# ziniuwan/maed

Hardware: AMD Instinct MI355X
Metric: video-clips/sec (BxT frames) train step (higher is better)
Workload: dtype bf16

## Files before the change

include/maed_hip.h:

```cpp
#ifndef MAED_HIP_H
#define MAED_HIP_H

#include <stddef.h>
#include <stdint.h>

#ifdef __cplusplus
extern "C" {
#endif

typedef enum { MAED_F32 = 0, MAED_BF16 = 1,
               MAED_F32X3 = 2, MAED_F32X6 = 3,
               MAED_F32X1 = 4 } maed_dtype;

typedef enum {
    MAED_OK = 0,
    MAED_ERR_ARG = -1,
    MAED_ERR_SHAPE = -2,
    MAED_ERR_ALIGN = -3,
    MAED_ERR_LAUNCH = -4,
    MAED_ERR_UNSUPPORTED = -5
} maed_status;

typedef enum {
    MAED_EPI_STORE = 0,
// ... 21 lines not shown
const char* maed_last_error(void);
int maed_version(void);

typedef enum {
    MAED_OPT_F32_MATMUL = 0,
    MAED_OPT_SIDE_STREAM = 1,
    MAED_OPT_TN_TARGET_WGS = 2,
    MAED_OPT_ABLATE = 3,
    MAED_OPT_GN_BWD_ONEPASS = 4,
    MAED_OPT_F32_BWD_X1 = 5,
    MAED_OPT_ST_FUSED = 6,
    MAED_OPT_CONV3X3_ROWS_WGS = 7,
    MAED_OPT_STEM_WGRAD_WGS = 8,
    MAED_OPT_LBS_FRAMES = 9,
    MAED_OPT_TN_DMA = 10,
    MAED_OPT_X3_PLANES = 11,
    MAED_OPT_X3_PLANES_LN = 12,
    MAED_OPT_SK = 13,
    MAED_OPT_SK_GRID = 14,
    MAED_OPT_TN_SK = 15,
    MAED_OPT_CONV3X3_NARROW_WGS = 16,
    MAED_OPT_CONV3X3_FRAME = 17,
    MAED_OPT_CONV3X3_WGRAD_TAPS = 18,
    MAED_OPT_COUNT
} maed_option;
int maed_init(int device);
int maed_device_faults(void);
int maed_device_faults_clear(void);
int maed_set_option(int key, int value);
int maed_get_option(int key);

int maed_layernorm_fwd(const float* x, int64_t x_row_stride, const float* gamma, const float* beta,
                       void* y, int dtype, float* mean, float* rstd,
                       int64_t rows, int C, float eps, void* stream);
int maed_layernorm_bwd(const void* dy, int dtype, const float* x, int64_t x_row_stride,
                       const float* gamma, const float* mean, const float* rstd,
                       const float* dres_in, float* dx_out, void* dx_twin, float* dgamma, float* dbeta,
                       int64_t rows, int C, void* stream);

int maed_gemm_nt(const void* A, int64_t lda, const void* B, int64_t ldb,
                 int64_t M, int64_t N, int64_t K, int dtype, int epilogue,
                 const float* bias, void* out, int64_t ldo, void* out2,
                 const void* aux, int64_t ldaux, int splitk, int impl, void* stream);

int maed_gemm_nt_planes(const void* a_hi, const void* a_lo, int64_t lda, const void* b_hi, const void* b_lo, int64_t ldb, int64_t M, int64_t N, int64_t K,
                        int epilogue, const float* bias, void* out, int64_t ldo, void* out2_bf16, const void* aux, int64_t ldaux, void* out_hi, void* out_lo,
// ... 162 lines not shown

int maed_loss_accl_fwd_bwd(const float* pred_kp3d, const float* gt_kp3d, int N, int T, float weight, double* loss, float* d_kp3d, void* stream);

typedef struct {
    const float* w;
    float* gw;
    const void* gout;
    int64_t dst_off;
    int64_t dst_t_off;
    int32_t O, I, KHW, fstart;
    int32_t gout_f32;
    int32_t pad_;
} maed_ws_conv;
int maed_weight_std_fwd(const void* conv_table, int n_convs, int n_filters, void* out, int dtype, float* stats, float eps, int transpose_tiles, void* stream);
int maed_weight_std_bwd(const void* conv_table, int n_convs, int n_filters, int dtype, const float* stats, float eps, void* stream);
int maed_groupnorm_fwd(const void* x, const void* residual, const float* gamma, const float* beta, void* y, double* sums,
                       uint8_t* relu_mask, int N, int HW, int C, float eps, int relu, int dtype, int sums_zeroed, void* stream);
int maed_groupnorm_fwd_twin(const void* x, const void* residual, const float* gamma, const float* beta, void* y, double* sums,
                            uint8_t* relu_mask, int N, int HW, int C, float eps, int relu, int sums_zeroed, void* twin_x, void* twin_y, void* stream);
#define MAED_GN_SYNC_WORDS 80
int maed_groupnorm_bwd(const void* x, const uint8_t* relu_mask, const void* dy, const double* sums, const float* gamma, const float* beta,
                       void* dx, void* dres, float* dgamma, float* dbeta, float* ab_scratch, int N, int HW, int C, float eps,
                       int relu, int dtype, int ab_zeroed, uint32_t* frame_sync, void* aux_stream, void* stream);
typedef struct { const float* ab; float* dgamma; float* dbeta; int N; int C; } maed_gn_affine_item;
int maed_gn_affine_grad_batch(const maed_gn_affine_item* items, int count, void* stream);

int maed_maxpool3s2_same_fwd(const void* x, void* y, uint8_t* idx, int N, int H, int W, int C, int dtype, void* stream);
int maed_maxpool3s2_same_bwd(const void* dy, const uint8_t* idx, void* dx, int N, int H, int W, int C, int dtype, void* stream);
int maed_gn_relu_maxpool3s2_fwd(const void* x, const float* gamma, const float* beta, void* y, uint8_t* idx, double* sums, int N, int H, int W, int C, float eps,
                                int dtype, int sums_zeroed, void* stream);
int maed_groupnorm_dual_fwd(const void* x, const float* gamma, const float* beta, double* sums, const void* res, const float* gamma2, const float* beta2,
                            double* sums2, void* y, uint8_t* relu_mask, int N, int HW, int C, float eps, float eps2, int dtype, int sums_zeroed,
                            int sums2_zeroed, void* stream);

int maed_stem_input(const float* x, void* y, int N, int C, int H, int W, int pad_top, int pad_bottom, int pad_left, int pad_right, int c_stride, int dtype,
                    void* stream);

int maed_conv3x3_wgrad_rows64_scratch_floats(int F, int H, int W, int Cin, int Cout);
int maed_conv3x3_wgrad_rows64(const void* dy, const void* x, float* dW, void* scratch, int F, int H, int W, int dtype, void* stream);

int maed_conv3x3_wgrad_taps_scratch_floats(int F, int H, int W, int Cin, int Cout, int stride, int Ho, int Wo);
int maed_conv3x3_wgrad_taps(const void* dy, const void* x, const void* zero_page, float* dW, void* scratch, int F, int H, int W, int Cin, int Cout, int stride,
                            int pad_top, int pad_left, int Ho, int Wo, int dtype, void* stream);

int maed_stem7x7s2_supported(int H, int W);
int maed_stem7x7s2_fwd(const void* xp, const void* w, void* wimg, void* y, double* gn_sums, int F, int H, int W, int dtype, void* stream);
// ... 81 lines not shown
```

maed_amd/_lib.py:

```python
import ctypes as C
import os

HERE = os.path.dirname(os.path.abspath(__file__))
LIB_PATH = os.environ.get("MAED_HIP_LIB") or os.path.join(HERE, "libmaed_hip.so")

F32, BF16 = 0, 1
F32X3, F32X6, F32X1 = 2, 3, 4
EPI_STORE, EPI_GELU, EPI_RESID_F32, EPI_MUL_DGELU, EPI_ATOMIC_F32, EPI_STORE_F32, EPI_TANH, EPI_ADD = range(8)
EPI_RESID_DROP_F32, EPI_GELU_DROP, EPI_MUL_DGELU_DROP = 8, 9, 10
DROP_GOLD, DROP_SITE = 0x9E3779B97F4A7C15, 0xD1B54A32D192ED03
IMPL_AUTO, IMPL_VALU, IMPL_MFMA = 0, 1, 2
IMPL_MFMA_256 = 6
IMPL_MFMA_LONG = 5
IMPL_MFMA_SK = 10
IMPL_X3, IMPL_X6, IMPL_X1 = 7, 8, 9
(OPT_F32_MATMUL, OPT_SIDE_STREAM, OPT_TN_TARGET_WGS, OPT_ABLATE, OPT_GN_BWD_ONEPASS, OPT_F32_BWD_X1, OPT_ST_FUSED, OPT_CONV3X3_ROWS_WGS, OPT_STEM_WGRAD_WGS,
 OPT_LBS_FRAMES, OPT_TN_DMA, OPT_X3_PLANES, OPT_X3_PLANES_LN, OPT_SK, OPT_SK_GRID, OPT_TN_SK, OPT_CONV3X3_NARROW_WGS, OPT_CONV3X3_FRAME, OPT_CONV3X3_WGRAD_TAPS) = range(19)

vp, i64, i32, f32 = C.c_void_p, C.c_int64, C.c_int, C.c_float


class GnAffineItem(C.Structure):
    _fields_ = [("ab", C.c_void_p), ("dgamma", C.c_void_p), ("dbeta", C.c_void_p), ("N", C.c_int), ("C", C.c_int)]


class BlockDims(C.Structure):
    _fields_ = [("F", i32), ("P", i32), ("C", i32), ("H", i32), ("T", i32), ("hidden", i32),
                ("dtype", i32), ("impl", i32), ("eps", f32)]


_PARAM_FIELDS = ["ln1_g", "ln1_b", "ln2_g", "ln2_b", "w_qkv", "w_ts", "w_proj", "w_fc1", "w_fc2",
                 "b_qkv", "b_ts", "b_proj", "b_fc1", "b_fc2", "wt_qkv", "wt_ts", "wt_proj", "wt_fc1", "wt_fc2"]
_GRAD_FIELDS = _PARAM_FIELDS[:14]


class BlockParams(C.Structure):
    _fields_ = [(n, vp) for n in _PARAM_FIELDS]


class BlockGrads(C.Structure):
# ... 76 lines not shown
    "maed_prof_collect": (i32, [C.POINTER(C.c_double), C.POINTER(i32)]),
    "maed_prof_flops": (i32, [C.POINTER(C.c_double)]),
    "maed_prof_records": (i32, [i32, C.POINTER(C.c_double), C.POINTER(C.c_double), C.POINTER(C.c_double), i32]),
    "maed_ktd_chain_fwd": (i32, [vp, vp, vp, i32, vp]),
    "maed_rot6d_pose_fwd": (i32, [vp, vp, vp, i64, vp]),
    "maed_smpl_lbs_fwd": (i32, [C.POINTER(SmplParams), vp, vp, vp, vp, vp, vp, i32, vp]),
    "maed_joint_regress_fwd": (i32, [vp, i32, vp, vp, i32, vp]),
    "maed_joint_regress_csr_fwd": (i32, [vp, vp, vp, i32, vp, vp, i32, vp]),
    "maed_smpl_joints_project_fwd": (i32, [vp, vp, vp, vp, vp, vp, vp, i32, vp, vp, i32, vp]),
    "maed_smpl_joints_project_bwd": (i32, [vp, vp, vp, vp, vp, vp, i64, vp, vp, vp, vp, i32, vp]),
    "maed_smpl_skin_bwd": (i32, [C.POINTER(SmplParams), vp, vp, vp, vp, vp, vp, vp, vp, vp, i32, vp]),
    "maed_smpl_skin_bwd_sparse": (i32, [C.POINTER(SmplParams), vp, vp, vp, i32, vp, vp, vp, vp, vp, vp, i32, vp]),
    "maed_smpl_chain_bwd": (i32, [C.POINTER(SmplParams), vp, vp, vp, vp, vp, vp, vp, i64, vp, vp, i32, vp]),
    "maed_rot6d_pose_bwd": (i32, [vp, vp, vp, i64, vp, i64, vp]),
    "maed_ktd_chain_bwd": (i32, [vp, vp, vp, vp, vp, vp, i64, vp, vp, i32, vp]),
    "maed_ktd_pack": (i32, [C.POINTER(KtdPtrs), i32, vp, vp, vp, vp]),
    "maed_ktd_unpack_add": (i32, [C.POINTER(KtdPtrs), i32, vp, vp, vp, vp]),
    "maed_loss_fwd_bwd": (i32, [vp, vp, i32, vp, vp, vp, vp, vp, i32, C.POINTER(LossWeights), vp, vp, vp, vp, vp, vp]),
    "maed_weight_std_fwd": (i32, [vp, i32, i32, vp, i32, vp, f32, i32, vp]),
    "maed_weight_std_bwd": (i32, [vp, i32, i32, i32, vp, f32, vp]),
    "maed_groupnorm_fwd": (i32, [vp, vp, vp, vp, vp, vp, vp, i32, i32, i32, f32, i32, i32, i32, vp]),
    "maed_groupnorm_fwd_twin": (i32, [vp, vp, vp, vp, vp, vp, vp, i32, i32, i32, f32, i32, i32, vp, vp, vp]),
    "maed_groupnorm_bwd": (i32, [vp, vp, vp, vp, vp, vp, vp, vp, vp, vp, vp, i32, i32, i32, f32, i32, i32, i32, vp, vp, vp]),
    "maed_gn_affine_grad_batch": (i32, [vp, i32, vp]),
    "maed_comm_load": (i32, [C.c_char_p]),
    "maed_comm_unique_id": (i32, [vp]),
    "maed_comm_init": (i32, [i32, i32, vp]),
    "maed_comm_allreduce_async": (i32, [vp, C.c_size_t, i32, vp]),
    "maed_comm_wait": (i32, [vp]),
    "maed_comm_world": (i32, []),
    "maed_comm_destroy": (i32, []),
    "maed_conv3x3_fwd": (i32, [vp, vp, vp, vp, i32, i32, i32, i32, i32, i32, i32, i32, i32, i32, vp, i32, i32, vp, vp]),
    "maed_conv1x1_fwd": (i32, [vp, i64, vp, i64, i64, i32, i32, vp, i64, i32, vp, i32, vp]),
    "maed_conv3x3_tapmask": (i32, [vp, i32, i32, i32, vp]),
    "maed_conv3x3_s2_dgrad": (i32, [vp, vp, vp, vp, i32, i32, i32, i32, i32, i32, i32, i32, i32, i32, vp]),
    "maed_conv3x3_s2_tables": (i32, [vp, vp, i32, i32, i32, i32, i32, i32, i32, vp]),
    "maed_conv3x3_s2_wgrad": (i32, [vp, vp, vp, vp, vp, vp, i32, i32, i32, i32, i32, i32, i32, i32, vp]),
    "maed_conv3x3_wgrad": (i32, [vp, vp, vp, vp, vp, i32, i32, i32, i32, i32, i32, vp]),
    "maed_eval_pose_errors": (i32, [vp, vp, i32, i32, vp, vp, vp, vp, vp]),
    "maed_similarity_transform": (i32, [vp, vp, i32, i32, vp, vp]),
    "maed_eval_accel": (i32, [vp, vp, i32, i32, vp, vp]),
    "maed_eval_vertex_error": (i32, [vp, vp, i32, i32, vp, vp]),
    "maed_maxpool3s2_same_fwd": (i32, [vp, vp, vp, i32, i32, i32, i32, i32, vp]),
    "maed_maxpool3s2_same_bwd": (i32, [vp, vp, vp, i32, i32, i32, i32, i32, vp]),
    "maed_gn_relu_maxpool3s2_fwd": (i32, [vp, vp, vp, vp, vp, vp, i32, i32, i32, i32, f32, i32, i32, vp]),
    "maed_groupnorm_dual_fwd": (i32, [vp, vp, vp, vp, vp, vp, vp, vp, vp, vp, i32, i32, i32, f32, f32, i32, i32, i32, vp]),
# ... 44 lines not shown
        handle = C.CDLL(LIB_PATH)
        for name, (res, args) in SIGNATURES.items():
            fn = getattr(handle, name)
            fn.restype, fn.argtypes = res, args
        _lib = handle
        apply_options(handle)
        _init_pending = True
    if _init_pending:
        import torch
        if torch.cuda.is_available() and torch.cuda.is_initialized():
            _init_pending = False
            check(_lib.maed_init(torch.cuda.current_device()), "maed_init")
    return _lib


_OPTIONS = {
    OPT_F32_MATMUL: {"exact": 0, "0": 0, "bf16x3": 1, "1": 1, "bf16x6": 2, "2": 2}[os.environ.get("MAED_F32_MATMUL", "exact")],
    OPT_SIDE_STREAM: int(os.environ.get("MAED_WGRAD_SIDE_STREAM", "1") == "1"),
    OPT_TN_TARGET_WGS: int(os.environ.get("MAED_TN_TARGET_WGS", "0")),
    OPT_ABLATE: int(os.environ.get("MAED_GEMM_ABLATE", "0")),
    OPT_F32_BWD_X1: int(os.environ.get("MAED_F32_BWD", "") == "bf16x1"),
    OPT_ST_FUSED: int(os.environ.get("MAED_ST_FUSED", "1")),
    OPT_GN_BWD_ONEPASS: int(os.environ.get("MAED_GN_BWD_ONEPASS", "1")),
    OPT_CONV3X3_ROWS_WGS: 0 if os.environ.get("MAED_CONV3X3_WGRAD_ROWS", "1") == "0" else int(os.environ.get("MAED_CONV3X3_ROWS_WGS", "256")),
    OPT_STEM_WGRAD_WGS: int(os.environ.get("MAED_STEM_WGS", "512")),
    OPT_LBS_FRAMES: int(os.environ.get("MAED_LBS_FB", "0")),
    OPT_TN_DMA: int(os.environ.get("MAED_TN_DMA", "1")),
    OPT_X3_PLANES: int(os.environ.get("MAED_X3_PLANES", "6")),
    OPT_SK: int(os.environ.get("MAED_SK", "1")),
    OPT_SK_GRID: int(os.environ.get("MAED_SK_GRID", "0")),
    OPT_CONV3X3_FRAME: int(os.environ.get("MAED_CONV3X3_FRAME", "1")),
    OPT_CONV3X3_WGRAD_TAPS: int(os.environ.get("MAED_CONV3X3_WGRAD_TAPS", "1")),
    OPT_CONV3X3_NARROW_WGS: int(os.environ.get("MAED_CONV3X3_NARROW_WGS", "0")),
    OPT_TN_SK: int(os.environ.get("MAED_TN_SK", "1")),
    OPT_X3_PLANES_LN: int(os.environ.get("MAED_X3_PLANES_LN", "0")),
}


def apply_options(handle):
    for k, v in _OPTIONS.items():
        if handle.maed_set_option(k, v) != 0:
            raise MaedHipError(f"maed_set_option({k}, {v}) failed")


def set_option(key, value):
    _OPTIONS[key] = int(value)
# ... 21 lines not shown
```

maed_amd/csrc/backbone.hip:

```cpp
#include "common.cuh"

struct WsConv {
    const float* w;
    float* gw;
    const void* gout;
    int64_t dst_off;
    int64_t dst_t_off;
    int32_t O, I, KHW, fstart;
    int32_t gout_f32, pad_;
};
#define WS_MAX_CONVS 64

__device__ __forceinline__ int ws_find_conv(const WsConv* __restrict__ tab, int n_convs, int fi) {
    int c = 0;
    for (int i = 1; i < n_convs; ++i) c = (fi >= tab[i].fstart) ? i : c;
    return c;
}

template <typename T>
__global__ __launch_bounds__(256) void ws_fwd_kernel(const WsConv* __restrict__ tab, int n_convs, int n_filters, T* __restrict__ out,
                                                     float* __restrict__ stats , float eps, int skip_transposed) {
    const int fi = blockIdx.x * 4 + (threadIdx.x >> 6), lane = threadIdx.x & 63;
    if (fi >= n_filters) return;
    const WsConv d = tab[ws_find_conv(tab, n_convs, fi)];
// ... 437 lines not shown
#define GN1_NT 512
template <typename T> struct GnChunk;
template <> struct GnChunk<bf16> { uint4 v; };
template <> struct GnChunk<float> { float4 a, b; };
__device__ __forceinline__ void gn_chunk_ld(const bf16* p, GnChunk<bf16>& c) { c.v = *reinterpret_cast<const uint4*>(p); }
__device__ __forceinline__ void gn_chunk_ld(const float* p, GnChunk<float>& c) { c.a = *reinterpret_cast<const float4*>(p); c.b = *reinterpret_cast<const float4*>(p + 4); }
__device__ __forceinline__ void gn_chunk_st(bf16* p, const GnChunk<bf16>& c) { *reinterpret_cast<uint4*>(p) = c.v; }
__device__ __forceinline__ void gn_chunk_st(float* p, const GnChunk<float>& c) { *reinterpret_cast<float4*>(p) = c.a; *reinterpret_cast<float4*>(p + 4) = c.b; }
__device__ __forceinline__ void gn_chunk_zero(GnChunk<bf16>& c) { c.v = make_uint4(0u, 0u, 0u, 0u); }
__device__ __forceinline__ void gn_chunk_zero(GnChunk<float>& c) { c.a = make_float4(0.f, 0.f, 0.f, 0.f); c.b = c.a; }
__device__ __forceinline__ void gn_chunk_get(const GnChunk<bf16>& c, float (&o)[8]) {
    o[0] = __uint_as_float(c.v.x << 16); o[1] = __uint_as_float(c.v.x & 0xffff0000u); o[2] = __uint_as_float(c.v.y << 16); o[3] = __uint_as_float(c.v.y & 0xffff0000u);
    o[4] = __uint_as_float(c.v.z << 16); o[5] = __uint_as_float(c.v.z & 0xffff0000u); o[6] = __uint_as_float(c.v.w << 16); o[7] = __uint_as_float(c.v.w & 0xffff0000u);
}
__device__ __forceinline__ void gn_chunk_get(const GnChunk<float>& c, float (&o)[8]) {
    o[0] = c.a.x; o[1] = c.a.y; o[2] = c.a.z; o[3] = c.a.w; o[4] = c.b.x; o[5] = c.b.y; o[6] = c.b.z; o[7] = c.b.w;
}
__device__ __forceinline__ void gn_chunk_put(GnChunk<bf16>& c, const float (&o)[8]) {
    c.v = make_uint4(pack_bf2(o[0], o[1]), pack_bf2(o[2], o[3]), pack_bf2(o[4], o[5]), pack_bf2(o[6], o[7]));
}
__device__ __forceinline__ void gn_chunk_put(GnChunk<float>& c, const float (&o)[8]) {
    c.a = make_float4(o[0], o[1], o[2], o[3]); c.b = make_float4(o[4], o[5], o[6], o[7]);
}
#define GN1_SYNC_WORDS 80
template <typename T, bool RELU, bool YMASK, int GPC, int CH, int NT>
__global__ __launch_bounds__(NT, 4) void gn_bwd_onepass_kernel(const T* __restrict__ x, const uint8_t* __restrict__ mask, const T* __restrict__ dy,
                                                                   const double* __restrict__ sums, const float* __restrict__ gamma, const float* __restrict__ beta,
                                                                   float* ab , T* __restrict__ dx, T* __restrict__ dres,
                                                                   uint32_t* sync , int HW, int C, float eps, int S,
                                                                   int rows_per_wg, int phase, int skew, uint32_t* fault ) {
    MAED_DYN_SHARED(float, lpart);
    __shared__ float lmu[GN_G], lrs[GN_G], lgrp[GN_G * 2], lb[GN_G], lk[GN_G];
    __shared__ int lfail;
    const int n = blockIdx.y, tid = threadIdx.x, cpg = C / GN_G;
    if (tid < GN_G) {
        const double cnt = (double)HW * cpg;
        const double m = sums[((int64_t)n * GN_G + tid) * 2] / cnt;
        double var = sums[((int64_t)n * GN_G + tid) * 2 + 1] / cnt - m * m;
        if (var < 0.0) var = 0.0;
        lmu[tid] = (float)m; lrs[tid] = (float)(1.0 / sqrt(var + (double)eps));
    }
    if (tid < GN_G * 2) lgrp[tid] = 0.f;
    if (tid == 0) lfail = 0;
    __syncthreads();
    const int cbn = C / 8, cb = tid % cbn, rsub = tid / cbn, rstep = NT / cbn;
    constexpr int JS = 8 / GPC;
// ... 82 lines not shown
    __syncthreads();
    float A[8], B[GPC], K[GPC];
    {
        float gg[8];
        ld8(gamma + cb * 8, gg);
#pragma unroll
        for (int j = 0; j < 8; ++j) A[j] = rs[j / JS] * gg[j];
#pragma unroll
        for (int q = 0; q < GPC; ++q) { B[q] = lb[g0 + q]; K[q] = lk[g0 + q]; }
    }
#pragma unroll
    for (int k = 0; k < CH; ++k) {
        const int r = r0 + rsub + k * rstep;
        if (r >= r1) continue;
        float v[8], d[8], o[8];
        gn_chunk_get(xr[k], v); gn_chunk_get(dr[k], d);
        if (dres) gn_chunk_st(dres + base + (int64_t)r * C, dr[k]);
#pragma unroll
        for (int j = 0; j < 8; ++j) o[j] = fmaf(A[j], d[j], -fmaf((v[j] - mu[j / JS]) * rs[j / JS], K[j / JS], B[j / JS]));
        GnChunk<T> oc;
        gn_chunk_put(oc, o);
        gn_chunk_st(dx + base + (int64_t)r * C, oc);
    }
}

static int gn_check(int C, int HW, const char* who) {
    MAED_CHECK_ARG(C % GN_G == 0 && C % 8 == 0 && C / 8 <= 256 && 256 % (C / 8) == 0, MAED_ERR_SHAPE, "%s: C=%d unsupported (need C%%32==0, C/8 a power of two <= 256)", who, C);
    MAED_CHECK_ARG(HW > 0, MAED_ERR_SHAPE, "%s: HW=%d", who, HW);
    return MAED_OK;
}
static int gn_rows_per_wg(int N, int HW, int C, int target_wgs = 2048) {
    const int tile = 256 / (C / 8);
    int chunks = (target_wgs + N - 1) / N;
    int rows = (HW + chunks - 1) / chunks;
    rows = (rows + tile - 1) / tile * tile;
    return rows < tile ? tile : rows;
}

static int groupnorm_fwd(const void* x, const void* residual, const float* gamma, const float* beta, void* y, double* sums,
                         uint8_t* relu_mask, int N, int HW, int C, float eps, int relu, int dtype, int sums_zeroed, void* twin_x, void* twin_y, void* stream) {
    MAED_CHECK_ARG(x && gamma && beta && y && sums, MAED_ERR_ARG, "groupnorm_fwd: null pointer");
    MAED_PROPAGATE(gn_check(C, HW, "groupnorm_fwd"));
    if (N <= 0) return MAED_OK;
    hipStream_t s = (hipStream_t)stream;
    const int rows = gn_rows_per_wg(N, HW, C);
    dim3 grid((HW + rows - 1) / rows, N);
// ... 27 lines not shown
    if (!sums_zeroed) MAED_HIP(hipMemsetAsync(sums, 0, (size_t)N * GN_G * 2 * sizeof(double), s), "groupnorm statistics: memset");
    MAED_DISPATCH_DTYPE(dtype, T, hipLaunchKernelGGL((gn_stats_kernel<T>), grid, dim3(256), 0, s, (const T*)x, sums, HW, C, rows));
    MAED_CHECK_LAUNCH(who);
    return MAED_OK;
}

extern "C" int maed_groupnorm_dual_fwd(const void* x, const float* gamma, const float* beta, double* sums, const void* res, const float* gamma2, const float* beta2,
                                       double* sums2, void* y, uint8_t* relu_mask, int N, int HW, int C, float eps, float eps2, int dtype, int sums_zeroed,
                                       int sums2_zeroed, void* stream) {
    MAED_CHECK_ARG(x && gamma && beta && sums && res && gamma2 && beta2 && sums2 && y, MAED_ERR_ARG, "groupnorm_dual_fwd: null pointer");
    MAED_PROPAGATE(gn_check(C, HW, "groupnorm_dual_fwd"));
    if (N <= 0) return MAED_OK;
    hipStream_t s = (hipStream_t)stream;
    MAED_PROPAGATE(gn_stats_if_needed(x, sums, N, HW, C, dtype, sums_zeroed, s, "groupnorm_dual_fwd"));
    MAED_PROPAGATE(gn_stats_if_needed(res, sums2, N, HW, C, dtype, sums2_zeroed, s, "groupnorm_dual_fwd"));
    const int rows = gn_rows_per_wg(N, HW, C);
    dim3 grid((HW + rows - 1) / rows, N);
    MAED_DISPATCH_DTYPE(dtype, T, hipLaunchKernelGGL((gn_apply_dual_kernel<T>), grid, dim3(256), 0, s, (const T*)x, sums, gamma, beta, (const T*)res, sums2, gamma2,
                                                      beta2, (T*)y, relu_mask, HW, C, eps, eps2, rows));
    MAED_CHECK_LAUNCH("groupnorm_dual_fwd");
    return MAED_OK;
}

extern "C" int maed_groupnorm_bwd(const void* x, const uint8_t* relu_mask, const void* dy, const double* sums, const float* gamma, const float* beta,
                                  void* dx, void* dres, float* dgamma, float* dbeta, float* ab_scratch, int N, int HW, int C, float eps,
                                  int relu, int dtype, int ab_zeroed, uint32_t* frame_sync, void* aux_stream, void* stream) {
    MAED_CHECK_ARG(x && dy && sums && gamma && beta && dx && ab_scratch, MAED_ERR_ARG, "groupnorm_bwd: null pointer");
    MAED_CHECK_ARG((dgamma != nullptr) == (dbeta != nullptr), MAED_ERR_ARG, "groupnorm_bwd: dgamma and dbeta go together (both NULL: the caller folds ab_scratch with maed_gn_affine_grad_batch)");
    MAED_CHECK_ARG(!(relu && dres) || relu_mask, MAED_ERR_ARG, "groupnorm_bwd: the forward's relu_mask is needed when a residual was added before the ReLU");
    MAED_PROPAGATE(gn_check(C, HW, "groupnorm_bwd"));
    if (N <= 0) return MAED_OK;
    hipStream_t s = (hipStream_t)stream;
    const int rows = gn_rows_per_wg(N, HW, C);
    dim3 grid((HW + rows - 1) / rows, N);
    const int rrows = gn_rows_per_wg(N, HW, C, 768);
    dim3 rgrid((HW + rrows - 1) / rrows, N);
    if (!ab_zeroed) MAED_HIP(hipMemsetAsync(ab_scratch, 0, (size_t)N * C * 2 * sizeof(float), s), "groupnorm_bwd: memset");
    const size_t lds = (size_t)(256 / (C / 8)) * 2 * C * sizeof(float);
    constexpr int defer = 1;
    const bool ymask = relu && relu_mask;
    const int cpg = C / GN_G, cbn1 = C / 8, ch1 = dtype == MAED_BF16 ? ((relu && !ymask) ? 7 : 8) : 4;
    int S1 = 0, rows1 = 0;
    const int nt1 = maed_opt(MAED_OPT_GN_BWD_ONEPASS) == 2 ? 256 : GN1_NT;
    uint32_t* const fault1 = maed_fault_word();
    bool onepass = frame_sync && maed_opt(MAED_OPT_GN_BWD_ONEPASS) && cpg >= 2 && cbn1 <= nt1 && !maed_fault_seen("groupnorm_bwd");
    if (onepass) {
        const int rstep = nt1 / cbn1, cap = ch1 * rstep;
        S1 = (HW + cap - 1) / cap;
        rows1 = (((HW + S1 - 1) / S1) + rstep - 1) / rstep * rstep;
        onepass = S1 <= 64;
    }
#define GN_RED(RELU_, YM_) hipLaunchKernelGGL((gn_bwd_reduce_kernel<T, RELU_, YM_>), rgrid, dim3(256), lds, s, (const T*)x, relu_mask, (const T*)dy, \
        sums, gamma, beta, ab_scratch, dgamma, dbeta, HW, C, eps, rrows, defer)
#define GN_APP(RES_, RELU_) hipLaunchKernelGGL((gn_bwd_apply_kernel<T, RES_, RELU_>), grid, dim3(256), 0, s, (const T*)x, relu_mask, (const T*)dy, \
        sums, ab_scratch, gamma, beta, (T*)dx, (T*)dres, HW, C, eps, rows)
#define GN_ONE4(RELU_, YM_, GPC_, CH_, PH_, NT_) hipLaunchKernelGGL((gn_bwd_onepass_kernel<T, RELU_, YM_, GPC_, CH_, NT_>), dim3(S1, N), dim3(NT_), lds1, s, (const T*)x, relu_mask, \
        (const T*)dy, sums, gamma, beta, ab_scratch, (T*)dx, (T*)dres, frame_sync, HW, C, eps, (maed_opt(MAED_OPT_GN_BWD_ONEPASS) == 3 ? 1 : S1), rows1, PH_, skew1, fault1)
#define GN_ONE3(RELU_, YM_, GPC_, CH_, PH_) do { if (nt1 == 256) GN_ONE4(RELU_, YM_, GPC_, CH_, PH_, 256); else GN_ONE4(RELU_, YM_, GPC_, CH_, PH_, GN1_NT); } while (0)
#define GN_ONE2(RELU_, YM_, CH_, PH_) do { if (cpg >= 8) GN_ONE3(RELU_, YM_, 1, CH_, PH_); else if (cpg == 4) GN_ONE3(RELU_, YM_, 2, CH_, PH_); else GN_ONE3(RELU_, YM_, 4, CH_, PH_); } while (0)
#define GN_ONE(PH_) do { constexpr int CH_ = sizeof(T) == 2 ? 8 : 4, CHM_ = sizeof(T) == 2 ? 7 : 4; \
        if (!relu) GN_ONE2(false, false, CH_, PH_); else if (ymask) GN_ONE2(true, true, CH_, PH_); else GN_ONE2(true, false, CHM_, PH_); } while (0)
    const size_t lds1 = (size_t)(nt1 / cbn1) * 2 * C * sizeof(float);
    const int opt1 = maed_opt(MAED_OPT_GN_BWD_ONEPASS);
    const int skew1 = (int64_t)S1 * N >= 1536 ? (opt1 >= 10 ? opt1 - 10 : 2) : 0;
    MAED_DISPATCH_DTYPE(dtype, T, {
        if (onepass) {
#ifdef MAED_HOSTSIM
            GN_ONE(1); GN_ONE(2);
#else
            GN_ONE(0);
#endif
        } else if (!relu) GN_RED(false, false); else if (ymask) GN_RED(true, true); else GN_RED(true, false);
        if (defer && dgamma) {
            hipStream_t sa = s;
            if (aux_stream) {
                MAED_PROPAGATE(maed_stream_fence(s, aux_stream));
                sa = (hipStream_t)aux_stream;
            }
            hipLaunchKernelGGL(gn_affine_grad_kernel, dim3((2 * C + 63) / 64, (N + 63) / 64), dim3(256), 0, sa, ab_scratch, dgamma, dbeta, N, C);
        }
        if (onepass) { }
        else if (ymask) GN_APP(true, true); else if (dres) GN_APP(true, false); else if (relu) GN_APP(false, true); else GN_APP(false, false);
    });
#undef GN_RED
#undef GN_APP
#undef GN_ONE
#undef GN_ONE2
#undef GN_ONE3
#undef GN_ONE4
    MAED_CHECK_LAUNCH("groupnorm_bwd");
    return MAED_OK;
}

template <typename T>
__global__ __launch_bounds__(256) void maxpool3s2_fwd_kernel(const T* __restrict__ x, T* __restrict__ y, uint8_t* __restrict__ idx, int N, int H, int W,
                                                             int C, int Ho, int Wo, int top, int left) {
    const int64_t i = (int64_t)blockIdx.x * 256 + threadIdx.x;
    const int cb = C / 8;
    if (i >= (int64_t)N * Ho * Wo * cb) return;
    const int c8 = (int)(i % cb) * 8;
    const int64_t pix = i / cb;
    const int wo = (int)(pix % Wo), ho = (int)((pix / Wo) % Ho), n = (int)(pix / ((int64_t)Wo * Ho));
    float m[8]; int am[8];
#pragma unroll
    for (int j = 0; j < 8; ++j) { m[j] = -INFINITY; am[j] = 0; }
    bool first = true;
    for (int kh = 0; kh < 3; ++kh) {
        const int h = 2 * ho - top + kh;
        if (h < 0 || h >= H) continue;
        for (int kw = 0; kw < 3; ++kw) {
            const int w = 2 * wo - left + kw;
            if (w < 0 || w >= W) continue;
// ... 249 lines not shown
```

maed_amd/csrc/options.hip:

```cpp
#include "common.cuh"
#include "gemm_x3.h"
#include <atomic>
#include <string.h>

static std::atomic<int> g_opt[MAED_OPT_COUNT] = {
    {0},
    {1},
    {0},
    {0},
    {1},
    {0},
    {1},
    {256},
    {512},
    {0},
    {1},
    {6},
    {0},
    {1},
    {0},
    {1},
    {0},
    {1},
    {1},
};

extern "C" int maed_init(int device) {
#ifndef MAED_HOSTSIM
    hipDeviceProp_t prop;
    if (hipGetDeviceProperties(&prop, device) != hipSuccess) { (void)hipGetLastError(); maed_set_error("init: no HIP device %d", device); return MAED_ERR_ARG; }
    if (!strstr(prop.gcnArchName, "gfx950")) {
        maed_set_error("init: device %d is %s; libmaed_hip is built for gfx950 (MI355X) only", device, prop.gcnArchName);
        return MAED_ERR_UNSUPPORTED;
    }
#else
    (void)device;
#endif
    (void)maed_fault_word();
#ifndef MAED_HOSTSIM
    if (maed_init_runtime() != MAED_OK) { maed_set_error("init: could not create the library's side streams / event rings"); return MAED_ERR_LAUNCH; }
#endif
    return MAED_OK;
}

static std::atomic<uint32_t*> g_fault{nullptr};
// ... 28 lines not shown
    return true;
}
extern "C" int maed_device_faults(void) {
    uint32_t* w = g_fault.load(std::memory_order_acquire);
    const int n = w ? (int)*(volatile uint32_t*)w : 0;
    if (n > 0)
        maed_set_error("%d frame-barrier timeout(s) on this device (workgroups of a frame were not co-resident: shared GPU / preemption); the affected results were "
                       "NaN-poisoned, the one-pass GroupNorm backward and the fused attentive addition run as their multi-launch forms from the next call on", n);
    return n;
}
extern "C" int maed_device_faults_clear(void) { uint32_t* w = g_fault.load(std::memory_order_acquire); if (w) *(volatile uint32_t*)w = 0; g_fault_told.store(0); return MAED_OK; }

extern "C" int maed_set_option(int key, int value) {
    MAED_CHECK_ARG(key >= 0 && key < MAED_OPT_COUNT, MAED_ERR_ARG, "set_option: unknown option %d", key);
    if (key == MAED_OPT_F32_MATMUL) MAED_CHECK_ARG(value >= 0 && value <= 2, MAED_ERR_ARG, "set_option: MAED_OPT_F32_MATMUL takes 0 (exact), 1 (bf16x3) or 2 (bf16x6)");
    if (key == MAED_OPT_TN_TARGET_WGS) MAED_CHECK_ARG(value == 0 || value >= 64, MAED_ERR_ARG, "set_option: MAED_OPT_TN_TARGET_WGS must be 0 (heuristic) or >= 64");
    if (key == MAED_OPT_CONV3X3_ROWS_WGS || key == MAED_OPT_STEM_WGRAD_WGS) MAED_CHECK_ARG(value >= 0 && value <= 65535, MAED_ERR_ARG, "set_option: workgroup count out of range");
    if (key == MAED_OPT_LBS_FRAMES) MAED_CHECK_ARG(value == 0 || value == 4 || value == 8 || value == 16, MAED_ERR_ARG, "set_option: MAED_OPT_LBS_FRAMES takes 0 (auto), 4, 8 or 16");
    if (key == MAED_OPT_X3_PLANES) MAED_CHECK_ARG(value == 0 || (value >= 2 && value <= 7 && value != 3), MAED_ERR_ARG, "set_option: MAED_OPT_X3_PLANES takes 0 (fp32 operands) or a kernel variant 2, 4, 5, 6, 7");
    if (key == MAED_OPT_SK) MAED_CHECK_ARG(value >= 0 && value <= 3, MAED_ERR_ARG, "set_option: MAED_OPT_SK takes 0 (off), 1 (heuristic), 2 (no K cuts) or 3 (always)");
    if (key == MAED_OPT_TN_SK) MAED_CHECK_ARG(value == 0 || value == 1, MAED_ERR_ARG, "set_option: MAED_OPT_TN_SK takes 0 or 1");
    if (key == MAED_OPT_SK_GRID) MAED_CHECK_ARG(value >= 0 && value <= 512, MAED_ERR_ARG, "set_option: MAED_OPT_SK_GRID takes 0 (one workgroup per CU) or a workgroup count <= 512");
    if (key == MAED_OPT_CONV3X3_WGRAD_TAPS) MAED_CHECK_ARG(value >= 0 && value <= 2 + 65535, MAED_ERR_ARG, "set_option: MAED_OPT_CONV3X3_WGRAD_TAPS takes 0, 1, 2 or 2 + a chunk count");
    g_opt[key].store(value, std::memory_order_relaxed);
    return MAED_OK;
}

extern "C" int maed_get_option(int key) {
    if (key < 0 || key >= MAED_OPT_COUNT) { maed_set_error("get_option: unknown option %d", key); return MAED_ERR_ARG; }
    return g_opt[key].load(std::memory_order_relaxed);
}

int maed_opt(int key) { return g_opt[key].load(std::memory_order_relaxed); }

int maed_x3_planes(void) {
    const int v = maed_opt(MAED_OPT_F32_MATMUL);
    return v == 1 ? 2 : v == 2 ? 3 : 0;
}
```

Before: 426.8.

## Add channel-slice single-kernel GroupNorm backward for small spatial bf16 layers

Adds a GroupNorm backward kernel where each workgroup owns a 64-channel slice of one frame. It holds all rows (HW ≤ 256) in registers, reduces the per-channel sums in LDS, and applies dx in the same launch. This removes the reduce/apply split, the ab memset, and the frame-barrier one-pass path for late ResNet stages. A new option, on by default, selects it when the grid has at least 256 workgroups. The cost is higher register pressure and lower occupancy per workgroup.

Result: no change. 426.2 (-0.1%).

```diff
diff --git a/include/maed_hip.h b/include/maed_hip.h
--- a/include/maed_hip.h
+++ b/include/maed_hip.h
@@ -67,6 +67,7 @@
     MAED_OPT_CONV3X3_NARROW_WGS = 16,
     MAED_OPT_CONV3X3_FRAME = 17,
     MAED_OPT_CONV3X3_WGRAD_TAPS = 18,
+    MAED_OPT_GN_BWD_SLICES = 19,
     MAED_OPT_COUNT
 } maed_option;
 int maed_init(int device);
@@ -275,6 +276,7 @@
 int maed_groupnorm_bwd(const void* x, const uint8_t* relu_mask, const void* dy, const double* sums, const float* gamma, const float* beta,
                        void* dx, void* dres, float* dgamma, float* dbeta, float* ab_scratch, int N, int HW, int C, float eps,
                        int relu, int dtype, int ab_zeroed, uint32_t* frame_sync, void* aux_stream, void* stream);
+int maed_groupnorm_bwd_form(int N, int HW, int C, int dtype, int has_frame_sync);
 typedef struct { const float* ab; float* dgamma; float* dbeta; int N; int C; } maed_gn_affine_item;
 int maed_gn_affine_grad_batch(const maed_gn_affine_item* items, int count, void* stream);
 
diff --git a/maed_amd/_lib.py b/maed_amd/_lib.py
--- a/maed_amd/_lib.py
+++ b/maed_amd/_lib.py
@@ -15,7 +15,8 @@
 IMPL_MFMA_SK = 10
 IMPL_X3, IMPL_X6, IMPL_X1 = 7, 8, 9
 (OPT_F32_MATMUL, OPT_SIDE_STREAM, OPT_TN_TARGET_WGS, OPT_ABLATE, OPT_GN_BWD_ONEPASS, OPT_F32_BWD_X1, OPT_ST_FUSED, OPT_CONV3X3_ROWS_WGS, OPT_STEM_WGRAD_WGS,
- OPT_LBS_FRAMES, OPT_TN_DMA, OPT_X3_PLANES, OPT_X3_PLANES_LN, OPT_SK, OPT_SK_GRID, OPT_TN_SK, OPT_CONV3X3_NARROW_WGS, OPT_CONV3X3_FRAME, OPT_CONV3X3_WGRAD_TAPS) = range(19)
+ OPT_LBS_FRAMES, OPT_TN_DMA, OPT_X3_PLANES, OPT_X3_PLANES_LN, OPT_SK, OPT_SK_GRID, OPT_TN_SK, OPT_CONV3X3_NARROW_WGS, OPT_CONV3X3_FRAME, OPT_CONV3X3_WGRAD_TAPS,
+ OPT_GN_BWD_SLICES) = range(20)
 
 vp, i64, i32, f32 = C.c_void_p, C.c_int64, C.c_int, C.c_float
 
@@ -138,6 +139,7 @@
     "maed_groupnorm_fwd": (i32, [vp, vp, vp, vp, vp, vp, vp, i32, i32, i32, f32, i32, i32, i32, vp]),
     "maed_groupnorm_fwd_twin": (i32, [vp, vp, vp, vp, vp, vp, vp, i32, i32, i32, f32, i32, i32, vp, vp, vp]),
     "maed_groupnorm_bwd": (i32, [vp, vp, vp, vp, vp, vp, vp, vp, vp, vp, vp, i32, i32, i32, f32, i32, i32, i32, vp, vp, vp]),
+    "maed_groupnorm_bwd_form": (i32, [i32, i32, i32, i32, i32]),
     "maed_gn_affine_grad_batch": (i32, [vp, i32, vp]),
     "maed_comm_load": (i32, [C.c_char_p]),
     "maed_comm_unique_id": (i32, [vp]),
@@ -228,6 +230,7 @@
     OPT_F32_BWD_X1: int(os.environ.get("MAED_F32_BWD", "") == "bf16x1"),
     OPT_ST_FUSED: int(os.environ.get("MAED_ST_FUSED", "1")),
     OPT_GN_BWD_ONEPASS: int(os.environ.get("MAED_GN_BWD_ONEPASS", "1")),
+    OPT_GN_BWD_SLICES: int(os.environ.get("MAED_GN_BWD_SLICES", "1")),
     OPT_CONV3X3_ROWS_WGS: 0 if os.environ.get("MAED_CONV3X3_WGRAD_ROWS", "1") == "0" else int(os.environ.get("MAED_CONV3X3_ROWS_WGS", "256")),
     OPT_STEM_WGRAD_WGS: int(os.environ.get("MAED_STEM_WGS", "512")),
     OPT_LBS_FRAMES: int(os.environ.get("MAED_LBS_FB", "0")),
diff --git a/maed_amd/csrc/backbone.hip b/maed_amd/csrc/backbone.hip
--- a/maed_amd/csrc/backbone.hip
+++ b/maed_amd/csrc/backbone.hip
@@ -483,6 +483,10 @@
 __device__ __forceinline__ void gn_chunk_put(GnChunk<float>& c, const float (&o)[8]) {
     c.a = make_float4(o[0], o[1], o[2], o[3]); c.b = make_float4(o[4], o[5], o[6], o[7]);
 }
+__device__ __forceinline__ uint32_t gn_pair_keep(uint32_t w, uint32_t b2) { return w & (((b2 & 1u) ? 0x0000ffffu : 0u) | ((b2 & 2u) ? 0xffff0000u : 0u)); }
+__device__ __forceinline__ void gn_chunk_keep(GnChunk<bf16>& c, uint32_t bits) {
+    c.v.x = gn_pair_keep(c.v.x, bits); c.v.y = gn_pair_keep(c.v.y, bits >> 2); c.v.z = gn_pair_keep(c.v.z, bits >> 4); c.v.w = gn_pair_keep(c.v.w, bits >> 6);
+}
 #define GN1_SYNC_WORDS 80
 template <typename T, bool RELU, bool YMASK, int GPC, int CH, int NT>
 __global__ __launch_bounds__(NT, 4) void gn_bwd_onepass_kernel(const T* __restrict__ x, const uint8_t* __restrict__ mask, const T* __restrict__ dy,
@@ -611,6 +615,124 @@
         gn_chunk_put(oc, o);
         gn_chunk_st(dx + base + (int64_t)r * C, oc);
     }
+}
+
+#define GNS_NT 256
+#define GNS_SLICE 64
+template <bool RELU, bool YMASK, int GPC, int CH>
+__global__ __launch_bounds__(GNS_NT, CH == 7 ? ((RELU && !YMASK) ? 3 : 4) : (YMASK ? 3 : 2))
+void gn_bwd_slice_kernel(const bf16* __restrict__ x, const uint8_t* __restrict__ mask, const bf16* __restrict__ dy, const double* __restrict__ sums,
+                         const float* __restrict__ gamma, const float* __restrict__ beta, float* __restrict__ ab , bf16* __restrict__ dx,
+                         bf16* __restrict__ dres, int HW, int C, float eps) {
+    __shared__ float lred[GNS_NT / 64][GNS_SLICE * 2];
+    __shared__ float lch[GNS_SLICE * 2];
+    __shared__ float lmu[GN_G], lrs[GN_G], lb[GN_G], lk[GN_G];
+    const int n = blockIdx.y, tid = threadIdx.x, cpg = C / GN_G, c0 = blockIdx.x * GNS_SLICE, ng = GNS_SLICE / cpg, gfirst = c0 / cpg;
+    if (tid < ng) {
+        const double cnt = (double)HW * cpg;
+        const double m = sums[((int64_t)n * GN_G + gfirst + tid) * 2] / cnt;
+        double var = sums[((int64_t)n * GN_G + gfirst + tid) * 2 + 1] / cnt - m * m;
+        if (var < 0.0) var = 0.0;
+        lmu[tid] = (float)m; lrs[tid] = (float)(1.0 / sqrt(var + (double)eps));
+    }
+    __syncthreads();
+    const int cb = tid & 7, rl = tid >> 3, cbn = C / 8;
+    constexpr int JS = 8 / GPC;
+    const int g0 = cb * 8 / cpg;
+    float mu[GPC], rs[GPC];
+#pragma unroll
+    for (int q = 0; q < GPC; ++q) { mu[q] = lmu[g0 + q]; rs[q] = lrs[g0 + q]; }
+    const int64_t fbase = ((int64_t)n * HW) * C + c0;
+    const uint32_t tbyte = (uint32_t)(rl * C + cb * 8) * 2u, moff = (uint32_t)(rl * cbn + cb);
+#define GNS_AT(p_, k_) ((decltype(p_))((const char*)((p_) + fbase + (int64_t)(k_) * 32 * C) + tbyte))
+    const uint8_t* const mrow = mask + ((int64_t)n * HW) * cbn + blockIdx.x * (GNS_SLICE / 8);
+
+    GnChunk<bf16> xr[CH], dr[CH];
+    uint32_t mb[(CH + 3) / 4];
+#pragma unroll
+    for (int k = 0; k < (CH + 3) / 4; ++k) mb[k] = 0u;
+#pragma unroll
+    for (int k = 0; k < CH; ++k) {
+        const int r = rl + k * 32;
+        if (r < HW) {
+            gn_chunk_ld(GNS_AT(x, k), xr[k]);
+            gn_chunk_ld(GNS_AT(dy, k), dr[k]);
+            if (RELU && YMASK) mb[k >> 2] |= (uint32_t)(mrow + (int64_t)k * 32 * cbn)[moff] << (8 * (k & 3));
+        } else { gn_chunk_zero(xr[k]); gn_chunk_zero(dr[k]); }
+    }
+    {
+        float sa[8], sb[8], ga[8], be[8];
+#pragma unroll
+        for (int j = 0; j < 8; ++j) { sa[j] = 0.f; sb[j] = 0.f; ga[j] = 0.f; be[j] = 0.f; }
+        if (RELU && !YMASK) { ld8(gamma + c0 + cb * 8, ga); ld8(beta + c0 + cb * 8, be); }
+#pragma unroll
+        for (int k = 0; k < CH; ++k) {
+            if (k * 32 >= HW) continue;
+            float v[8], d[8];
+            gn_chunk_get(xr[k], v);
+#pragma unroll
+            for (int j = 0; j < 8; ++j) v[j] = (v[j] - mu[j / JS]) * rs[j / JS];
+            if (RELU) {
+                uint32_t bits = (mb[k >> 2] >> (8 * (k & 3))) & 0xffu;
+                if (!YMASK) {
+#pragma unroll
+                    for (int j = 0; j < 8; ++j) bits |= (fmaf(v[j], ga[j], be[j]) > 0.f ? 1u : 0u) << j;
+                }
+                gn_chunk_keep(dr[k], bits);
+            }
+            gn_chunk_get(dr[k], d);
+#pragma unroll
+            for (int j = 0; j < 8; ++j) { sa[j] += d[j]; sb[j] = fmaf(d[j], v[j], sb[j]); }
+        }
+#pragma unroll
+        for (int j = 0; j < 8; ++j)
+#pragma unroll
+            for (int m = 8; m < 64; m <<= 1) { sa[j] += __shfl_xor(sa[j], m, 64); sb[j] += __shfl_xor(sb[j], m, 64); }
+        if ((tid & 63) < 8) {
+            float* mine = &lred[tid >> 6][cb * 16];
+#pragma unroll
+            for (int j = 0; j < 8; ++j) { mine[2 * j] = sa[j]; mine[2 * j + 1] = sb[j]; }
+        }
+    }
+    __syncthreads();
+    if (tid >= GNS_NT - GNS_SLICE * 2) {
+        const uint32_t i = (uint32_t)tid - (GNS_NT - GNS_SLICE * 2);
+        const float t = (lred[0][i] + lred[1][i]) + (lred[2][i] + lred[3][i]);
+        lch[i] = t;
+        (ab + ((int64_t)n * C + c0) * 2)[i] = t;
+    }
+    __syncthreads();
+    if (tid < ng * 2) {
+        const int g = tid >> 1, w = tid & 1;
+        float p = 0.f;
+        for (int c = g * cpg; c < (g + 1) * cpg; ++c) p = fmaf(gamma[c0 + c], lch[2 * c + w], p);
+        const float cnt = (float)(HW * cpg);
+        (w ? lk : lb)[g] = lrs[g] * (p / cnt);
+    }
+    __syncthreads();
+    float A[8], B[GPC], K[GPC];
+    {
+        float gg[8];
+        ld8(gamma + c0 + cb * 8, gg);
+#pragma unroll
+        for (int j = 0; j < 8; ++j) A[j] = rs[j / JS] * gg[j];
+#pragma unroll
+        for (int q = 0; q < GPC; ++q) { B[q] = lb[g0 + q]; K[q] = lk[g0 + q]; }
+    }
+#pragma unroll
+    for (int k = 0; k < CH; ++k) {
+        const int r = rl + k * 32;
+        if (r >= HW) continue;
+        float v[8], d[8], o[8];
+        gn_chunk_get(xr[k], v); gn_chunk_get(dr[k], d);
+        if (dres) gn_chunk_st(GNS_AT(dres, k), dr[k]);
+#pragma unroll
+        for (int j = 0; j < 8; ++j) o[j] = fmaf(A[j], d[j], -fmaf((v[j] - mu[j / JS]) * rs[j / JS], K[j / JS], B[j / JS]));
+        GnChunk<bf16> oc;
+        gn_chunk_put(oc, o);
+        gn_chunk_st(GNS_AT(dx, k), oc);
+    }
+#undef GNS_AT
 }
 
 static int gn_check(int C, int HW, const char* who) {
@@ -684,6 +806,28 @@
     return MAED_OK;
 }
 
+#define GNS_MIN_WGS 256
+static int gn_bwd_form(int N, int HW, int C, int dtype, bool has_frame_sync, int relu, bool ymask, int* nt1_out, int* S1_out, int* rows1_out) {
+    const int cpg = C / GN_G, sopt = maed_opt(MAED_OPT_GN_BWD_SLICES);
+    if (sopt && dtype == MAED_BF16 && C % GNS_SLICE == 0 && cpg >= 2 && GNS_SLICE % cpg == 0 && HW <= 256 && (sopt == 2 || (int64_t)N * (C / GNS_SLICE) >= GNS_MIN_WGS))
+        return 2;
+    const int cbn1 = C / 8, ch1 = dtype == MAED_BF16 ? ((relu && !ymask) ? 7 : 8) : 4;
+    const int nt1 = maed_opt(MAED_OPT_GN_BWD_ONEPASS) == 2 ? 256 : GN1_NT;
+    if (!(has_frame_sync && maed_opt(MAED_OPT_GN_BWD_ONEPASS) && cpg >= 2 && cbn1 <= nt1 && !maed_fault_seen("groupnorm_bwd"))) return 0;
+    const int rstep = nt1 / cbn1, cap = ch1 * rstep;
+    const int S1 = (HW + cap - 1) / cap;
+    if (S1 > 64) return 0;
+    if (nt1_out) *nt1_out = nt1;
+    if (S1_out) *S1_out = S1;
+    if (rows1_out) *rows1_out = (((HW + S1 - 1) / S1) + rstep - 1) / rstep * rstep;
+    return 1;
+}
+extern "C" int maed_groupnorm_bwd_form(int N, int HW, int C, int dtype, int has_frame_sync) {
+    MAED_CHECK_ARG(dtype == MAED_F32 || dtype == MAED_BF16, MAED_ERR_ARG, "groupnorm_bwd_form: dtype %d", dtype);
+    MAED_PROPAGATE(gn_check(C, HW, "groupnorm_bwd_form"));
+    return gn_bwd_form(N, HW, C, dtype, has_frame_sync != 0, 1, false, nullptr, nullptr, nullptr);
+}
+
 extern "C" int maed_groupnorm_bwd(const void* x, const uint8_t* relu_mask, const void* dy, const double* sums, const float* gamma, const float* beta,
                                   void* dx, void* dres, float* dgamma, float* dbeta, float* ab_scratch, int N, int HW, int C, float eps,
                                   int relu, int dtype, int ab_zeroed, uint32_t* frame_sync, void* aux_stream, void* stream) {
@@ -697,21 +841,15 @@
     dim3 grid((HW + rows - 1) / rows, N);
     const int rrows = gn_rows_per_wg(N, HW, C, 768);
     dim3 rgrid((HW + rrows - 1) / rrows, N);
-    if (!ab_zeroed) MAED_HIP(hipMemsetAsync(ab_scratch, 0, (size_t)N * C * 2 * sizeof(float), s), "groupnorm_bwd: memset");
+    const bool ymask = relu && relu_mask;
+    const int cpg = C / GN_G, cbn1 = C / 8;
+    int S1 = 0, rows1 = 0, nt1 = GN1_NT;
+    const int form = gn_bwd_form(N, HW, C, dtype, frame_sync != nullptr, relu, ymask, &nt1, &S1, &rows1);
+    const bool onepass = form == 1, slices = form == 2;
+    if (!ab_zeroed && !slices) MAED_HIP(hipMemsetAsync(ab_scratch, 0, (size_t)N * C * 2 * sizeof(float), s), "groupnorm_bwd: memset");
     const size_t lds = (size_t)(256 / (C / 8)) * 2 * C * sizeof(float);
     constexpr int defer = 1;
-    const bool ymask = relu && relu_mask;
-    const int cpg = C / GN_G, cbn1 = C / 8, ch1 = dtype == MAED_BF16 ? ((relu && !ymask) ? 7 : 8) : 4;
-    int S1 = 0, rows1 = 0;
-    const int nt1 = maed_opt(MAED_OPT_GN_BWD_ONEPASS) == 2 ? 256 : GN1_NT;
     uint32_t* const fault1 = maed_fault_word();
-    bool onepass = frame_sync && maed_opt(MAED_OPT_GN_BWD_ONEPASS) && cpg >= 2 && cbn1 <= nt1 && !maed_fault_seen("groupnorm_bwd");
-    if (onepass) {
-        const int rstep = nt1 / cbn1, cap = ch1 * rstep;
-        S1 = (HW + cap - 1) / cap;
-        rows1 = (((HW + S1 - 1) / S1) + rstep - 1) / rstep * rstep;
-        onepass = S1 <= 64;
-    }
 #define GN_RED(RELU_, YM_) hipLaunchKernelGGL((gn_bwd_reduce_kernel<T, RELU_, YM_>), rgrid, dim3(256), lds, s, (const T*)x, relu_mask, (const T*)dy, \
         sums, gamma, beta, ab_scratch, dgamma, dbeta, HW, C, eps, rrows, defer)
 #define GN_APP(RES_, RELU_) hipLaunchKernelGGL((gn_bwd_apply_kernel<T, RES_, RELU_>), grid, dim3(256), 0, s, (const T*)x, relu_mask, (const T*)dy, \
@@ -722,11 +860,18 @@
 #define GN_ONE2(RELU_, YM_, CH_, PH_) do { if (cpg >= 8) GN_ONE3(RELU_, YM_, 1, CH_, PH_); else if (cpg == 4) GN_ONE3(RELU_, YM_, 2, CH_, PH_); else GN_ONE3(RELU_, YM_, 4, CH_, PH_); } while (0)
 #define GN_ONE(PH_) do { constexpr int CH_ = sizeof(T) == 2 ? 8 : 4, CHM_ = sizeof(T) == 2 ? 7 : 4; \
         if (!relu) GN_ONE2(false, false, CH_, PH_); else if (ymask) GN_ONE2(true, true, CH_, PH_); else GN_ONE2(true, false, CHM_, PH_); } while (0)
+#define GN_SLC4(RELU_, YM_, GPC_, CH_) hipLaunchKernelGGL((gn_bwd_slice_kernel<RELU_, YM_, GPC_, CH_>), dim3(C / GNS_SLICE, N), dim3(GNS_NT), 0, s, (const bf16*)x, relu_mask, \
+        (const bf16*)dy, sums, gamma, beta, ab_scratch, (bf16*)dx, (bf16*)dres, HW, C, eps)
+#define GN_SLC3(RELU_, YM_, GPC_) do { if (HW <= 7 * 32) GN_SLC4(RELU_, YM_, GPC_, 7); else GN_SLC4(RELU_, YM_, GPC_, 8); } while (0)
+#define GN_SLC2(RELU_, YM_) do { if (cpg >= 8) GN_SLC3(RELU_, YM_, 1); else if (cpg == 4) GN_SLC3(RELU_, YM_, 2); else GN_SLC3(RELU_, YM_, 4); } while (0)
+#define GN_SLC() do { if (!relu) GN_SLC2(false, false); else if (ymask) GN_SLC2(true, true); else GN_SLC2(true, false); } while (0)
     const size_t lds1 = (size_t)(nt1 / cbn1) * 2 * C * sizeof(float);
     const int opt1 = maed_opt(MAED_OPT_GN_BWD_ONEPASS);
     const int skew1 = (int64_t)S1 * N >= 1536 ? (opt1 >= 10 ? opt1 - 10 : 2) : 0;
     MAED_DISPATCH_DTYPE(dtype, T, {
-        if (onepass) {
+        if (slices) {
+            GN_SLC();
+        } else if (onepass) {
 #ifdef MAED_HOSTSIM
             GN_ONE(1); GN_ONE(2);
 #else
@@ -741,7 +886,7 @@
             }
             hipLaunchKernelGGL(gn_affine_grad_kernel, dim3((2 * C + 63) / 64, (N + 63) / 64), dim3(256), 0, sa, ab_scratch, dgamma, dbeta, N, C);
         }
-        if (onepass) { }
+        if (onepass || slices) { }
         else if (ymask) GN_APP(true, true); else if (dres) GN_APP(true, false); else if (relu) GN_APP(false, true); else GN_APP(false, false);
     });
 #undef GN_RED
@@ -750,6 +895,10 @@
 #undef GN_ONE2
 #undef GN_ONE3
 #undef GN_ONE4
+#undef GN_SLC
+#undef GN_SLC2
+#undef GN_SLC3
+#undef GN_SLC4
     MAED_CHECK_LAUNCH("groupnorm_bwd");
     return MAED_OK;
 }
diff --git a/maed_amd/csrc/options.hip b/maed_amd/csrc/options.hip
--- a/maed_amd/csrc/options.hip
+++ b/maed_amd/csrc/options.hip
@@ -21,6 +21,7 @@
     {0},
     {1},
     {0},
+    {1},
     {1},
     {1},
 };
@@ -95,6 +96,7 @@
     if (key == MAED_OPT_TN_SK) MAED_CHECK_ARG(value == 0 || value == 1, MAED_ERR_ARG, "set_option: MAED_OPT_TN_SK takes 0 or 1");
     if (key == MAED_OPT_SK_GRID) MAED_CHECK_ARG(value >= 0 && value <= 512, MAED_ERR_ARG, "set_option: MAED_OPT_SK_GRID takes 0 (one workgroup per CU) or a workgroup count <= 512");
     if (key == MAED_OPT_CONV3X3_WGRAD_TAPS) MAED_CHECK_ARG(value >= 0 && value <= 2 + 65535, MAED_ERR_ARG, "set_option: MAED_OPT_CONV3X3_WGRAD_TAPS takes 0, 1, 2 or 2 + a chunk count");
+    if (key == MAED_OPT_GN_BWD_SLICES) MAED_CHECK_ARG(value >= 0 && value <= 2, MAED_ERR_ARG, "set_option: MAED_OPT_GN_BWD_SLICES takes 0 (never), 1 (where the grid fills the chip) or 2 (wherever the shape qualifies)");
     g_opt[key].store(value, std::memory_order_relaxed);
     return MAED_OK;
 }
```
